# relife957/FastApriori

Measured on AMD Instinct MI355X. Metric: itemsets/sec (mining wall-clock), T10I4D100M min_sup=0.001, higher is better.
Workload: dtype int32/uint64-bitmap (exact integer counts); 1 GPU; model=T10I4D100M, global_batch=100000000, parallelism=dp1, n_itemsets=33139, min_count=100000

## Files before the change

csrc/hip/fa_hip.h:

```cpp
#pragma once
#include <hip/hip_runtime.h>
#include <stdint.h>

#define FA_API extern "C" __attribute__((visibility("default")))

#define FA_LAUNCH_RET() return (int)hipGetLastError()

namespace fa {

constexpr int kWave = 64;

__device__ __forceinline__ int lane_id() { return (int)(threadIdx.x & 63); }

__device__ __forceinline__ uint32_t popc64_acc(uint64_t x, uint32_t acc) {
  return acc + (uint32_t)__popc((uint32_t)x) + (uint32_t)__popc((uint32_t)(x >> 32));
}

__device__ __forceinline__ int wave_scan_incl_dpp(int v) {
  const int lane = (int)(threadIdx.x & 63);
  const int r = lane & 15;
  int t;
  t = __builtin_amdgcn_update_dpp(0, v, 0x111, 0xf, 0xf, false); if (r >= 1) v += t;
  t = __builtin_amdgcn_update_dpp(0, v, 0x112, 0xf, 0xf, false); if (r >= 2) v += t;
  t = __builtin_amdgcn_update_dpp(0, v, 0x114, 0xf, 0xf, false); if (r >= 4) v += t;
  t = __builtin_amdgcn_update_dpp(0, v, 0x118, 0xf, 0xf, false); if (r >= 8) v += t;
  t = __builtin_amdgcn_update_dpp(0, v, 0x142, 0xa, 0xf, false); if ((lane & 31) >= 16) v += t;
  t = __builtin_amdgcn_update_dpp(0, v, 0x143, 0xc, 0xf, false); if (lane >= 32) v += t;
  return v;
}

__device__ __forceinline__ int wave_last(int v) { return __builtin_amdgcn_readlane(v, 63); }

__device__ __forceinline__ uint32_t wave_sum_u32(uint32_t v) {
#pragma unroll
  for (int o = 32; o > 0; o >>= 1) v += __shfl_xor(v, o, 64);
  return v;
}

__device__ __forceinline__ unsigned long long wave_sum_u64(unsigned long long v) {
#pragma unroll
  for (int o = 32; o > 0; o >>= 1) v += __shfl_xor(v, o, 64);
  return v;
}

__device__ __forceinline__ int64_t wave_scan_incl_i64(int64_t v) {
  const int lane = (int)(threadIdx.x & 63);
#pragma unroll
  for (int o = 1; o < 64; o <<= 1) {
    const int64_t t = __shfl_up(v, o, 64);
    if (lane >= o) v += t;
  }
  return v;
}

__device__ __forceinline__ int wave_scan_incl(int v) { return wave_scan_incl_dpp(v); }
__device__ __forceinline__ int64_t wave_scan_incl(int64_t v) { return wave_scan_incl_i64(v); }
__device__ __forceinline__ int wave_sum(int v) { return (int)wave_sum_u32((uint32_t)v); }
__device__ __forceinline__ uint32_t wave_sum(uint32_t v) { return wave_sum_u32(v); }
__device__ __forceinline__ int64_t wave_sum(int64_t v) { return (int64_t)wave_sum_u64((unsigned long long)v); }


template <int W, int N, typename T, typename A>
__device__ __forceinline__ void wg_wave_prefix(const T (&x)[N], int src, T* scratch, A (&before)[N], A (&total)[N]) {
  const int lane = (int)(threadIdx.x & 63), w = (int)(threadIdx.x >> 6);
#pragma unroll
  for (int j = 0; j < N; ++j)
    if (lane == src) scratch[j * W + w] = x[j];
  __syncthreads();
#pragma unroll
  for (int j = 0; j < N; ++j) {
    A bef = 0, tot = 0;
#pragma unroll 4
    for (int k = 0; k < W; ++k) {
      const A t = (A)scratch[j * W + k];
      bef += k < w ? t : (A)0;
      tot += t;
    }
    before[j] = bef;
    total[j] = tot;
  }
}

template <int W, int N, typename T, typename A>
__device__ __forceinline__ void wg_scan_excl(const T (&v)[N], T* scratch, A (&excl)[N], A (&total)[N]) {
  T incl[N];
#pragma unroll
  for (int j = 0; j < N; ++j) incl[j] = wave_scan_incl(v[j]);
  wg_wave_prefix<W>(incl, 63, scratch, excl, total);
#pragma unroll
  for (int j = 0; j < N; ++j) excl[j] += (A)incl[j] - (A)v[j];
}

template <int W, typename T, typename A>
__device__ __forceinline__ A wg_scan_excl(T v, T* scratch, A& total) {
  const T v1[1] = {v};
  A e[1], t[1];
  wg_scan_excl<W>(v1, scratch, e, t);
  total = t[0];
  return e[0];
}

template <int W, int N, typename T>
__device__ __forceinline__ void wg_sum(const T (&v)[N], T* scratch, T (&total)[N]) {
  T s[N], before[N];
#pragma unroll
  for (int j = 0; j < N; ++j) s[j] = wave_sum(v[j]);
  wg_wave_prefix<W>(s, 0, scratch, before, total);
}

template <int W, typename T>
__device__ __forceinline__ T wg_sum(T v, T* scratch) {
  const T v1[1] = {v};
  T t[1];
  wg_sum<W>(v1, scratch, t);
  return t[0];
}

template <int W, int N, typename T, class Load, class Store>
__device__ __forceinline__ void wg_scan_chunks(int64_t n, int64_t (&carry)[N], T* scratch, Load&& load,
                                               Store&& store) {
  for (int64_t b0 = 0; b0 < n; b0 += 64 * W) {
    const int64_t i = b0 + threadIdx.x;
    T v[N];
#pragma unroll
    for (int j = 0; j < N; ++j) v[j] = 0;
    if (i < n) load(i, v);
    int64_t before[N], total[N];
    wg_scan_excl<W>(v, scratch, before, total);
#pragma unroll
    for (int j = 0; j < N; ++j) {
      before[j] += carry[j];
      carry[j] += total[j];
    }
    if (i < n) store(i, before, v);
    __syncthreads();
  }
}

template <int W, typename T, class Load, class Store>
__device__ __forceinline__ int64_t wg_scan_chunks(int64_t n, int64_t carry, T* scratch, Load&& load, Store&& store) {
  int64_t c[1] = {carry};
  wg_scan_chunks<W, 1>(
      n, c, scratch, [&](int64_t i, T (&v)[1]) { v[0] = load(i); },
      [&](int64_t i, const int64_t (&before)[1], const T (&v)[1]) { store(i, before[0], v[0]); });
  return c[0];
}

__device__ __forceinline__ void wave_lds_sync() {
  __builtin_amdgcn_wave_barrier();
  __asm__ __volatile__("" ::: "memory");
}

template <int U>
__device__ __forceinline__ void window_starts(unsigned long long* words, int srel, int q0,
                                              unsigned long long (&S)[U]) {
  const int lane = (int)(threadIdx.x & 63);
  if (lane < U) words[lane] = 0ull;
  wave_lds_sync();
  const int b = srel - q0;
  if (b >= 0 && b < 64 * U) atomicOr(&words[b >> 6], 1ull << (b & 63));
  wave_lds_sync();
#pragma unroll
  for (int u = 0; u < U; ++u) S[u] = words[u];
  wave_lds_sync();
}

__device__ __forceinline__ unsigned long long lanes_le_mask() {
  const int lane = (int)(threadIdx.x & 63);
  return lane == 63 ? ~0ull : ((2ull << lane) - 1);
}

__device__ __forceinline__ uint32_t xcd_remap(uint32_t orig, uint32_t nwg) {
  const uint32_t nx = 8;
  if (nwg < nx) return orig;
  uint32_t q = nwg / nx, r = nwg % nx, xcd = orig % nx;
  uint32_t base = xcd < r ? xcd * (q + 1) : r * (q + 1) + (xcd - r) * q;
  return base + orig / nx;
}

__device__ __forceinline__ int cmp_skip(const int32_t* __restrict__ a, const int32_t* __restrict__ s, int k,
                                        int p) {
  for (int i = 0, j = 0; i < k - 1; ++i, ++j) {
    if (j == p) ++j;
    const int32_t x = a[i], y = s[j];
    if (x != y) return x < y ? -1 : 1;
  }
  return 0;
}

struct DlDesc;

}

FA_API int fa_hip_dl_plan(const fa::DlDesc* desc, int L, long long* ctl, int F1, int32_t* item_map, void* rec,
                          int64_t max_pieces, int32_t* part, int64_t part_cap, int32_t* gpre, int64_t gpre_cap,
                          int sw, hipStream_t st);
FA_API int fa_hip_count_slab_rec_cls(const int64_t* roff, const int32_t* ranks, const int32_t* src, int64_t ncols,
                                     const int32_t* item_map, int F1, int n_used, const int32_t* gpre,
                                     const void* rec, int G, int C, const int32_t* wword, uint32_t* out, int sw,
                                     int n_wg, const uint64_t* bm, int64_t Wp, hipStream_t st,
                                     const int32_t* bm_rows, const int32_t* g_dev, int cls);
```

csrc/hip/prep.hip:

```cpp
#include "fa_hip.h"
#include "../host/fa_limits.h"

namespace fa {


template <bool kLds, bool kVec>
__global__ __launch_bounds__(256) void k_histogram(const int32_t* __restrict__ items, int64_t nnz,
                                                   int32_t V, int nrep, uint32_t* __restrict__ counts) {
  extern __shared__ uint32_t sh[];
  uint32_t* mine = sh;
  if (kLds) {
    for (int i = threadIdx.x; i < V * nrep; i += blockDim.x) sh[i] = 0;
    mine = sh + (nrep > 1 ? (threadIdx.x >> 6) % nrep : 0) * V;
    __syncthreads();
  }
  auto add = [&](int32_t v) {
    if (kLds) atomicAdd(&mine[v], 1u); else atomicAdd(&counts[v], 1u);
  };
  const int64_t stride = (int64_t)gridDim.x * blockDim.x;
  const int64_t gid = (int64_t)blockIdx.x * blockDim.x + threadIdx.x;
  const int64_t n4 = kVec ? (nnz >> 2) : 0;
  const int4* it4 = reinterpret_cast<const int4*>(items);
  for (int64_t i = gid; i < n4; i += stride) {
    int4 v = it4[i];
// ... 369 lines not shown
      for (int k = 0; k < 4; ++k) v[k] = v[k] >= 0 ? lut[v[k]] : -1;
#pragma unroll
      for (int k = 0; k < 4; ++k)
        if (v[k] >= 0) atomicOr(&b[v[k] >> 6], 1ull << (v[k] & 63));
    }
    wave_lds_sync();
    int base = 0;
    for (int m = 0; m < M; ++m) {
      const int widx = lane + 64 * m;
      unsigned long long word = b[widx];
      b[widx] = 0;
      const int c = __popcll(word);
      const int incl = wave_scan_incl_dpp(c);
      int64_t pos = o + base + incl - c;
      base += wave_last(incl);
      while (word) {
        ranks[pos++] = widx * 64 + (__ffsll((long long)word) - 1);
        word &= word - 1;
      }
    }
    wave_lds_sync();
  }
}

__device__ __forceinline__ uint64_t dmix64(uint64_t z) {
  z += 0x9E3779B97F4A7C15ull;
  z = (z ^ (z >> 30)) * 0xBF58476D1CE4E5B9ull;
  z = (z ^ (z >> 27)) * 0x94D049BB133111EBull;
  return z ^ (z >> 31);
}

__global__ __launch_bounds__(256) void k_row_hash(const int64_t* __restrict__ roff,
                                                  const int32_t* __restrict__ ranks, int64_t T,
                                                  int64_t* __restrict__ h1, int64_t* __restrict__ h2) {
  const int64_t x = (int64_t)blockIdx.x * blockDim.x + threadIdx.x;
  if (x >= T) return;
  uint64_t a = 0x243F6A8885A308D3ull, b = 0x13198A2E03707344ull;
  const int64_t s = roff[x], e = roff[x + 1];
  for (int64_t i = s; i < e; ++i) {
    uint64_t r = (uint32_t)ranks[i];
    a = dmix64(a ^ r);
    b = dmix64(b + r * 0xD6E8FEB86659FD93ull);
  }
  a = dmix64(a ^ (uint64_t)(e - s));
  h1[x] = (int64_t)(a >> 1);
  h2[x] = (int64_t)(b >> 1);
}

constexpr int kCmpProbeLen = 16;

constexpr uint32_t kNoSlot = 0xFFFFFFFFu;
constexpr int kProbeRange = 1 << 16;

__global__ __launch_bounds__(256) void k_dedup_probe(const int64_t* __restrict__ roff,
                                                     const int32_t* __restrict__ ranks,
                                                     const int64_t* __restrict__ T_dev, int64_t n_max,
                                                     uint32_t* __restrict__ slots, uint32_t* __restrict__ part) {
  const int64_t n = min(T_dev[0], n_max);
  const int64_t x = (int64_t)blockIdx.x * 256 + threadIdx.x;
  uint32_t slot = kNoSlot;
  if (x < n) {
    const int64_t s = roff[x], e = roff[x + 1];
    const int L = (int)(e - s);
    if (L <= kCmpProbeLen) {
      uint32_t v[kCmpProbeLen];
#pragma unroll
      for (int j = 0; j < kCmpProbeLen; ++j) v[j] = j < L ? (uint32_t)ranks[s + j] : 0u;
      uint64_t a = 0x243F6A8885A308D3ull;
#pragma unroll
      for (int j = 0; j < kCmpProbeLen; ++j)
        if (j < L) a = dmix64(a ^ (uint64_t)v[j]);
      a = dmix64(a ^ (uint64_t)L);
      slot = (uint32_t)((a >> 1) & (kProbeBits - 1));
    }
  }
  if (x < n_max) slots[x] = slot;
  __shared__ uint32_t wsum[4];
  const uint32_t c = wg_sum<4>(slot != kNoSlot ? 1u : 0u, wsum);
  if (threadIdx.x == 0) part[blockIdx.x] = c;
}

__global__ __launch_bounds__(1024) void k_probe_count(const uint32_t* __restrict__ slots, int64_t n_max,
                                                      const uint32_t* __restrict__ part, int nparts,
                                                      unsigned long long* __restrict__ out) {
  __shared__ uint32_t bits[kProbeRange / 32];
  __shared__ uint32_t wsum[2 * 16];
  for (int i = threadIdx.x; i < kProbeRange / 32; i += 1024) bits[i] = 0u;
  __syncthreads();
  const uint32_t lo = (uint32_t)blockIdx.x * kProbeRange;
  const uint4* s4 = reinterpret_cast<const uint4*>(slots);
  const int64_t n4 = n_max >> 2;
  auto mark = [&](uint32_t v) {
    const uint32_t d = v - lo;
    if (d < (uint32_t)kProbeRange) atomicOr(&bits[d >> 5], 1u << (d & 31));
  };
  constexpr int U = 8;
  int64_t i = threadIdx.x;
  for (; i + (U - 1) * 1024 < n4; i += U * 1024) {
    uint4 v[U];
#pragma unroll
    for (int k = 0; k < U; ++k) v[k] = s4[i + k * 1024];
#pragma unroll
    for (int k = 0; k < U; ++k) { mark(v[k].x); mark(v[k].y); mark(v[k].z); mark(v[k].w); }
  }
  for (; i < n4; i += 1024) {
    const uint4 v = s4[i];
    mark(v.x); mark(v.y); mark(v.z); mark(v.w);
  }
  for (int64_t j = (n4 << 2) + threadIdx.x; j < n_max; j += 1024) mark(slots[j]);
  __syncthreads();
  uint32_t c = 0, h = 0;
  for (int i = threadIdx.x; i < kProbeRange / 32; i += 1024) c += __popc(bits[i]);
  if (blockIdx.x == 0)
    for (int i = threadIdx.x; i < nparts; i += 1024) h += part[i];
  const uint32_t ch[2] = {c, h};
  uint32_t t[2];
  wg_sum<16>(ch, wsum, t);
  if (threadIdx.x == 0) {
    if (t[0]) atomicAdd(out, (unsigned long long)t[0]);
    if (blockIdx.x == 0) out[1] = t[1];
  }
}

__global__ __launch_bounds__(256) void k_build_bitmaps(
    const int64_t* __restrict__ roff, const int32_t* __restrict__ ranks, const int32_t* __restrict__ src,
    int64_t ncols, int32_t F1, int64_t Wp, int WT, int R, uint64_t* __restrict__ bm,
    const int32_t* __restrict__ item_map, const int32_t* __restrict__ used) {
  extern __shared__ uint32_t tile[];
  const int hw = 2 * WT;
  const int u0 = blockIdx.y * R;
  const int u1 = min(F1, u0 + R);
  const int nr = u1 - u0;
  const int r0 = item_map ? used[u0] : u0;
  const int r1 = item_map ? (u1 < F1 ? used[u1] : 0x7FFFFFFF) : u1;
  for (int i = threadIdx.x; i < nr * hw; i += blockDim.x) tile[i] = 0;
  __syncthreads();
  const int64_t c0 = (int64_t)blockIdx.x * WT * 64;
  for (int j = threadIdx.x; j < WT * 64; j += blockDim.x) {
    const int64_t c = c0 + j;
    if (c >= ncols) break;
    const int64_t row = src ? (int64_t)src[c] : c;
    if (row < 0) continue;
    int64_t s = roff[row];
    const int64_t e = roff[row + 1];
    int64_t lo = s, hi = e;
    while (lo < hi) {
      int64_t mid = (lo + hi) >> 1;
      if (ranks[mid] < r0) lo = mid + 1; else hi = mid;
    }
    const uint32_t bit = 1u << (j & 31);
    const int word = j >> 5;
    for (int64_t i = lo; i < e; ++i) {
      const int r = ranks[i];
      if (r >= r1) break;
      const int u = item_map ? item_map[r] : r;
      if (u >= 0) atomicOr(&tile[(u - u0) * hw + word], bit);
    }
  }
  __syncthreads();
  uint32_t* out = reinterpret_cast<uint32_t*>(bm);
  const int64_t base = c0 >> 5;
  for (int i = threadIdx.x; i < nr * hw; i += blockDim.x) {
    const int r = i / hw, w = i - r * hw;
    out[(int64_t)(u0 + r) * (2 * Wp) + base + w] = tile[i];
  }
}

__device__ __forceinline__ unsigned long long lane_range(int lo, int hi) {
  const unsigned long long h = hi >= 64 ? ~0ull : ((1ull << hi) - 1);
  const unsigned long long l = lo >= 64 ? ~0ull : ((1ull << lo) - 1);
  return hi > lo ? (h & ~l) : 0ull;
}

struct TrimWave {
  int64_t base;
  int n;
  int srel, erel;
};

__device__ __forceinline__ TrimWave trim_wave_setup(const int64_t* __restrict__ roff, int64_t row0, int64_t T) {
  const int lane = threadIdx.x & 63;
  TrimWave tw;
  tw.base = roff[row0];
  const int64_t end = roff[min(row0 + 64, T)];
  tw.n = (int)(end - tw.base);
  tw.srel = (int)(roff[min(row0 + lane, T)] - tw.base);
  tw.erel = (int)(roff[min(row0 + lane + 1, T)] - tw.base);
  return tw;
}

template <bool kLdsAlive>
__global__ __launch_bounds__(256) void k_trim_scan_count(const int64_t* __restrict__ roff,
                                                         const int32_t* __restrict__ ranks, int64_t T,
                                                         const int8_t* __restrict__ alive, int F1, int min_len,
                                                         const int32_t* __restrict__ wrow, int32_t* __restrict__ cnt,
                                                         int32_t* __restrict__ bk_rows, int32_t* __restrict__ bk_nnz) {
  extern __shared__ int8_t al[];
  __shared__ int wtot[4];
  if (kLdsAlive)
    for (int i = threadIdx.x; i < F1; i += blockDim.x) al[i] = alive[i];
  __syncthreads();
  const int8_t* A = kLdsAlive ? al : alive;
  const int lane = threadIdx.x & 63;
  const int64_t row0 = (int64_t)blockIdx.x * 256 + (threadIdx.x & ~63);
  const int64_t row = row0 + lane;
  int c = 0;
  if (row0 < T) {
    const TrimWave tw = trim_wave_setup(roff, row0, T);
    constexpr int U = 8;
    for (int p0 = 0; p0 < tw.n; p0 += 64 * U) {
      int32_t r[U];
#pragma unroll
      for (int u = 0; u < U; ++u) {
        const int p = p0 + 64 * u + lane;
        r[u] = p < tw.n ? ranks[tw.base + p] : 0;
      }
#pragma unroll
      for (int u = 0; u < U; ++u) {
        const int q0 = p0 + 64 * u;
        const unsigned long long b = __ballot(q0 + lane < tw.n && A[r[u]] != 0);
        c += __popcll(b & lane_range(max(tw.srel - q0, 0), min(max(tw.erel - q0, 0), 64)));
      }
    }
  }
  const bool keep = row < T && c >= min_len && (!wrow || wrow[row] > 0);
  if (row < T) cnt[row] = keep ? c : -1;
  int tr, tn;
  (void)wg_scan_excl<4>(keep ? 1 : 0, wtot, tr);
  __syncthreads();
  (void)wg_scan_excl<4>(keep ? c : 0, wtot, tn);
  __syncthreads();
  if (threadIdx.x == 0) { bk_rows[blockIdx.x] = tr; bk_nnz[blockIdx.x] = tn; }
}

template <bool kLdsAlive>
__global__ __launch_bounds__(256) void k_trim_emit(const int64_t* __restrict__ roff, const int32_t* __restrict__ ranks,
                                                   const int8_t* __restrict__ alive, int F1, int64_t T,
                                                   const int32_t* __restrict__ cnt, const int64_t* __restrict__ base_rows,
                                                   const int64_t* __restrict__ base_nnz, int64_t* __restrict__ nroff,
                                                   int32_t* __restrict__ nranks, int32_t* __restrict__ kept,
                                                   int64_t* __restrict__ hist) {
  extern __shared__ int8_t al[];
  __shared__ uint32_t hs[kTrimHist];
  __shared__ unsigned long long sw[4 * 4];
  __shared__ int wtot[4];
  if (kLdsAlive)
    for (int i = threadIdx.x; i < F1; i += blockDim.x) al[i] = alive[i];
  hs[threadIdx.x] = 0;
  const int8_t* A = kLdsAlive ? al : alive;
  const int lane = threadIdx.x & 63;
  const int64_t row0 = (int64_t)blockIdx.x * 256 + (threadIdx.x & ~63);
  const int64_t row = row0 + lane;
  const int32_t c = row < T ? cnt[row] : -1;
  const bool keep = c >= 0;
  int nk, nn;
  const int rk = wg_scan_excl<4>(keep ? 1 : 0, wtot, nk);
  __syncthreads();
  const int ok = wg_scan_excl<4>(keep ? c : 0, wtot, nn);
  __syncthreads();
  const int64_t obase = base_nnz[blockIdx.x] + ok;
  if (keep) {
    nroff[base_rows[blockIdx.x] + rk] = obase;
    kept[base_rows[blockIdx.x] + rk] = (int32_t)row;
    atomicAdd(&hs[min(c, kTrimHist - 1)], 1u);
  }
  if (row0 < T && __ballot(keep) != 0ull) {
    const TrimWave tw = trim_wave_setup(roff, row0, T);
    int64_t nxt = keep ? obase : -1;
    unsigned long long* words = sw + (threadIdx.x >> 6) * 4;
    const unsigned long long le = lanes_le_mask();
    int cs = 0;
    constexpr int U = 4;
    for (int p0 = 0; p0 < tw.n; p0 += 64 * U) {
      int32_t r[U];
#pragma unroll
      for (int u = 0; u < U; ++u) {
        const int p = p0 + 64 * u + lane;
        r[u] = p < tw.n ? ranks[tw.base + p] : 0;
      }
      unsigned long long S[U];
      window_starts<U>(words, tw.srel, p0, S);
#pragma unroll
      for (int u = 0; u < U; ++u) {
        const int q0 = p0 + 64 * u, p = q0 + lane;
        const bool a = p < tw.n && A[r[u]] != 0;
        const unsigned long long B = __ballot(a);
        const unsigned long long sle = S[u] & le;
        const int owner = cs + __popcll(sle) - 1;
        const int rs = sle ? 63 - __clzll(sle) : 0;
        const int64_t dst = __shfl(nxt, owner & 63, 64);
        if (a && dst >= 0) nranks[dst + __popcll(B & lane_range(rs, lane))] = r[u];
        if (nxt >= 0) nxt += __popcll(B & lane_range(max(tw.srel - q0, 0), min(max(tw.erel - q0, 0), 64)));
        cs += __popcll(S[u]);
      }
    }
  }
  __syncthreads();
  if (hist && hs[threadIdx.x])
    atomicAdd((unsigned long long*)&hist[(blockIdx.x & (kTrimStripes - 1)) * kTrimHist + threadIdx.x], (unsigned long long)hs[threadIdx.x]);
}


constexpr int kCmpPer = kCmpSpan / 256;
__device__ __forceinline__ bool cmp_stage(uint32_t* buf, const int32_t* __restrict__ items,
                                          const int32_t* __restrict__ lut, int64_t base, int64_t n_in) {
  if (n_in > kCmpSpan) return false;
  int32_t v[kCmpPer];
#pragma unroll
  for (int k = 0; k < kCmpPer; ++k) {
    const int64_t i = threadIdx.x + k * 256;
    v[k] = i < n_in ? items[base + i] : 0;
  }
#pragma unroll
  for (int k = 0; k < kCmpPer; ++k) {
    const int64_t i = threadIdx.x + k * 256;
    if (i < n_in) v[k] = lut[v[k]];
  }
#pragma unroll
  for (int k = 0; k < kCmpPer; ++k) {
    const int64_t i = threadIdx.x + k * 256;
    if (i < n_in) buf[i] = v[k] < 0 ? 0xFFFFFFFFu : (uint32_t)v[k];
  }
  return true;
}

constexpr int kCmpN = 16;
constexpr int kCmpMid = 64;

__device__ __forceinline__ bool cmp_mid(bool kept, int64_t L, bool staged) {
  const bool cand = kept && staged && L > kCmpN && L <= kCmpMid;
  const unsigned long long m = __ballot(cand);
  return cand && __popcll(m & (lanes_le_mask() >> 1)) < kCmpMidPerWave;
}

template <int KMAX>
__device__ __forceinline__ void wave_sort2(uint32_t& a, uint32_t& b) {
  const int lane = threadIdx.x & 63;
#pragma unroll
  for (int k = 2; k <= KMAX; k <<= 1) {
#pragma unroll
    for (int j = k >> 1; j > 0; j >>= 1) {
      const uint32_t oa = (uint32_t)__shfl_xor((int)a, j, 64);
      const uint32_t ob = (uint32_t)__shfl_xor((int)b, j, 64);
      const bool up = k == KMAX || (lane & k) == 0;
      const bool keep_min = up == ((lane & j) == 0);
      a = keep_min ? min(a, oa) : max(a, oa);
      b = keep_min ? min(b, ob) : max(b, ob);
    }
  }
}

__device__ __forceinline__ int nth_bit(unsigned long long m, int i) {
  for (; i > 0; --i) m &= m - 1;
  return __builtin_ctzll(m);
}

__device__ __forceinline__ unsigned long long blk_inc(uint32_t v) {
  return v == 0xFFFFFFFFu ? 0ull : 1ull << ((v >> 8) << 3);
}

__device__ __forceinline__ void cmp_block_totals(unsigned long long pc, int nb, int32_t* __restrict__ aggb) {
  __shared__ int bs[kCmpMaxNB][4];
  const int w = threadIdx.x >> 6, lane = threadIdx.x & 63;
#pragma unroll
  for (int b = 0; b < kCmpMaxNB; ++b) {
    if (b >= nb) break;
    const int t = wave_last(wave_scan_incl_dpp((int)((pc >> (8 * b)) & 255)));
    if (lane == 0) bs[b][w] = t;
  }
  __syncthreads();
  if ((int)threadIdx.x < nb)
    aggb[(int64_t)threadIdx.x * gridDim.x + blockIdx.x] =
        bs[threadIdx.x][0] + bs[threadIdx.x][1] + bs[threadIdx.x][2] + bs[threadIdx.x][3];
}

__global__ __launch_bounds__(256) void k_cmp_agg(const int64_t* __restrict__ off, const int32_t* __restrict__ items,
                                                 const int32_t* __restrict__ lut, int64_t n,
                                                 int32_t* __restrict__ agg, uint32_t* __restrict__ hist,
                                                 int32_t* __restrict__ aggb, int nb) {
  __shared__ uint32_t buf[kCmpSpan];
  __shared__ uint32_t lh[kCmpHist];
  __shared__ int sh[8];
  const int64_t r0 = (int64_t)blockIdx.x * 256, r1 = min(n, r0 + 256);
  const int64_t r = r0 + threadIdx.x;
  lh[threadIdx.x] = 0;
  const int64_t base = off[r0], n_in = off[r1] - base;
  const int64_t s = r < r1 ? off[r] : 0, e = r < r1 ? off[r + 1] : 0;
  const bool staged = cmp_stage(buf, items, lut, base, n_in);
  __syncthreads();
  int c = 0;
  unsigned long long pc = 0;
  for (int64_t i = s; i < e; ++i) {
    const uint32_t v = staged ? buf[i - base] : (uint32_t)lut[items[i]];
    c += v != 0xFFFFFFFFu;
    if (aggb) pc += blk_inc(v);
  }
  const int kept = c >= 2;
  if (aggb) cmp_block_totals(kept ? pc : 0ull, nb, aggb);
  const int kc[2] = {kept, kept ? c : 0};
  int ex[2], tot[2];
  wg_scan_excl<4>(kc, sh, ex, tot);
  if (kept) atomicAdd(&lh[min(c, kCmpHist - 1)], 1u);
  const bool mid = cmp_mid(kept, e - s, staged);
  const unsigned long long ob = __ballot(kept && e - s > kCmpN && !mid);
  __shared__ int ov_w[4];
  const int ovn[1] = {(int)__popcll(ob)};
  int ovp[1], ovt[1];
  wg_wave_prefix<4>(ovn, 0, ov_w, ovp, ovt);
  if (threadIdx.x == 0) {
    agg[3 * blockIdx.x] = tot[0]; agg[3 * blockIdx.x + 1] = tot[1];
    agg[3 * blockIdx.x + 2] = ovt[0];
  }
  if (lh[threadIdx.x]) atomicAdd(&hist[(blockIdx.x & (kCmpStripes - 1)) * kCmpHist + threadIdx.x], lh[threadIdx.x]);
}

__global__ __launch_bounds__(256) void k_cmp_emit(const int64_t* __restrict__ off, const int32_t* __restrict__ items,
                                                  const int32_t* __restrict__ lut, int64_t n,
                                                  const int64_t* __restrict__ pre_rows,
                                                  const int64_t* __restrict__ pre_items,
                                                  const int64_t* __restrict__ pre_over,
                                                  int32_t* __restrict__ kept_out, int64_t* __restrict__ roff,
                                                  int32_t* __restrict__ ranks, int32_t* __restrict__ over,
                                                  uint8_t* __restrict__ bcnt, int nb,
                                                  const int64_t* __restrict__ preb, uint8_t* __restrict__ lr,
                                                  int64_t lr_cap, int64_t* __restrict__ lbase,
                                                  int64_t* __restrict__ ovb) {
  constexpr int N = kCmpN;
  __shared__ uint32_t buf[kCmpSpan];
  __shared__ int sh[8];
  extern __shared__ int32_t tabx[];
  __shared__ int64_t wgb[kCmpMaxNB];
  const bool blk = bcnt != nullptr;
  const int64_t r0 = (int64_t)blockIdx.x * 256, r1 = min(n, r0 + 256);
  const int64_t r = r0 + threadIdx.x;
  const int64_t base = off[r0], n_in = off[r1] - base;
  const int64_t s = r < r1 ? off[r] : 0, e = r < r1 ? off[r + 1] : 0;
  const int64_t xr0 = pre_rows[blockIdx.x], obase = pre_items[blockIdx.x];
  const bool staged = cmp_stage(buf, items, lut, base, n_in);
  __syncthreads();
  const int64_t L = e - s;
  uint32_t a[N];
  int c = 0;
  unsigned long long pc = 0;
  if (L <= N) {
#pragma unroll
    for (int j = 0; j < N; ++j) {
      uint32_t v = 0xFFFFFFFFu;
      if (j < L) v = staged ? buf[s - base + j] : (uint32_t)lut[items[s + j]];
      a[j] = v;
      c += v != 0xFFFFFFFFu;
      if (blk) pc += blk_inc(v);
    }
  } else {
    for (int64_t i = s; i < e; ++i) {
      const uint32_t v = staged ? buf[i - base] : (uint32_t)lut[items[i]];
      c += v != 0xFFFFFFFFu;
      if (blk) pc += blk_inc(v);
    }
  }
  const int kept = c >= 2;
  const bool mid = cmp_mid(kept, L, staged);
  const int ov = kept && L > N && !mid;
  const int kc[2] = {kept, kept ? c : 0};
  int ex[2], tot[2];
  wg_scan_excl<4>(kc, sh, ex, tot);
  const int ea = ex[0], eb = ex[1], tb = tot[1];
  __shared__ int ov_w[4];
  const int w = threadIdx.x >> 6;
  const unsigned long long ob = __ballot(ov);
  const int ovn[1] = {(int)__popcll(ob)};
  int64_t ovp[1], ovt[1];
  wg_wave_prefix<4>(ovn, 0, ov_w, ovp, ovt);
  const int64_t ov_base = pre_over[blockIdx.x];
  const int64_t xk = xr0 + ea;
  int64_t ovi = -1;
  if (kept) {
    kept_out[xk] = (int32_t)r;
    roff[xk + 1] = obase + eb + c;
    if (ov) {
      ovi = ov_base + ovp[0] + __popcll(ob & (lanes_le_mask() >> 1));
      over[ovi] = (int32_t)xk;
    }
  }
  const bool mine = kept && L <= N;
  if (mine) bitonic_regs<N>(a);
  if (blk) {
    const int64_t bld = pre_rows[gridDim.x];
    const unsigned long long pk = kept ? pc : 0ull;
    const unsigned long long fpre = (pk << 8) * 0x0101010101010101ull;
    __shared__ int bs2[kCmpMaxNB][4];
    const int lane_ = threadIdx.x & 63;
    int exb[kCmpMaxNB];
#pragma unroll
    for (int b = 0; b < kCmpMaxNB; ++b) {
      exb[b] = 0;
      if (b < nb) {
        const int cb = (int)((pk >> (8 * b)) & 255);
        const int incl = wave_scan_incl_dpp(cb);
        exb[b] = incl - cb;
        if (lane_ == 63) bs2[b][w] = incl;
      }
    }
    if (lr && (int)threadIdx.x < nb) wgb[threadIdx.x] = preb[(int64_t)threadIdx.x * gridDim.x + blockIdx.x];
    __syncthreads();
#pragma unroll
    for (int b = 0; b < kCmpMaxNB; ++b) {
      if (b < nb) {
        for (int k = 0; k < w; ++k) exb[b] += bs2[b][k];
        if (kept) bcnt[(int64_t)b * bld + xk] = (uint8_t)(pk >> (8 * b));
        if (lr) {
          const int t = exb[b] - (int)((fpre >> (8 * b)) & 255);
          tabx[threadIdx.x * nb + b] = t;
          if (kept && (xk & 63) == 0) lbase[(int64_t)b * ((bld + 63) >> 6) + (xk >> 6)] = wgb[b] + exb[b];
          if (ovi >= 0) ovb[ovi * nb + b] = wgb[b] + t;
        }
      }
    }
    if (lr && mine) {
#pragma unroll
      for (int j = 0; j < N; ++j) {
        if (j < c) {
          const int b = (int)(a[j] >> 8);
          lr[wgb[b] + (int64_t)(tabx[threadIdx.x * nb + b] + j)] = (uint8_t)a[j];
        }
      }
    }
  }
  const int lane = threadIdx.x & 63;
  const unsigned long long m32 = __ballot(mid && L <= 32), m64 = __ballot(mid && L > 32);
  const int n32 = __popcll(m32), s32 = (n32 + 1) >> 1, nslot = s32 + __popcll(m64);
  auto slot_row = [&](int t) -> int {
    if (t < s32) {
      const int i = 2 * t + (lane >> 5);
      return i < n32 ? nth_bit(m32, i) : -1;
    }
    return t < nslot ? nth_bit(m64, t - s32) : -1;
  };
  uint32_t midv[kCmpMidPerWave];
#pragma unroll
  for (int t = 0; t < kCmpMidPerWave; ++t) {
    midv[t] = 0xFFFFFFFFu;
    if (t < nslot) {
      const int rw = slot_row(t);
      const int src = rw < 0 ? 0 : rw;
      const int idx = t < s32 ? (lane & 31) : lane;
      const int rs = __shfl((int)(s - base), src, 64);
      const int rl = __shfl((int)L, src, 64);
      if (rw >= 0 && idx < rl) midv[t] = buf[rs + idx];
    }
  }
#pragma unroll
  for (int t = 0; t < kCmpMidPerWave; t += 2) {
    if (t < nslot) {
      if (t + 1 < s32) {
        wave_sort2<32>(midv[t], midv[t + 1]);
      } else if (t >= s32) {
        wave_sort2<64>(midv[t], midv[t + 1]);
      } else {
        uint32_t none = 0xFFFFFFFFu;
        wave_sort2<32>(midv[t], none);
        if (t + 1 < nslot) wave_sort2<64>(midv[t + 1], none);
      }
    }
  }
  __syncthreads();
  if (staged && tb <= kCmpSpan) {
    if (mine) {
#pragma unroll
      for (int j = 0; j < N; ++j)
        if (j < c) buf[eb + j] = a[j];
    }
    {
#pragma unroll
      for (int t = 0; t < kCmpMidPerWave; ++t) {
        if (t < nslot) {
          const int rw = slot_row(t);
          const int src = rw < 0 ? 0 : rw;
          const int idx = t < s32 ? (lane & 31) : lane;
          const int rc = __shfl(c, src, 64), reb = __shfl(eb, src, 64);
          const bool in = rw >= 0 && idx < rc;
          if (in) {
            buf[reb + idx] = midv[t];
            if (lr) {
              const int b = (int)(midv[t] >> 8);
              lr[wgb[b] + (int64_t)(tabx[(w * 64 + rw) * nb + b] + idx)] = (uint8_t)midv[t];
            }
          }
        }
      }
    }
    __syncthreads();
    for (int i = threadIdx.x; i < tb; i += blockDim.x) ranks[obase + i] = (int32_t)buf[i];
  } else if (mine) {
#pragma unroll
    for (int j = 0; j < N; ++j)
      if (j < c) ranks[obase + eb + j] = (int32_t)a[j];
  }
}
__global__ __launch_bounds__(256) void k_block_counts_rows(const int64_t* __restrict__ roff,
                                                           const int32_t* __restrict__ ranks,
                                                           const int32_t* __restrict__ rows, int64_t nrows,
                                                           uint8_t* __restrict__ bcnt, int64_t bld, int nb,
                                                           const int8_t* __restrict__ flags) {
  const int64_t i = (int64_t)blockIdx.x * blockDim.x + threadIdx.x;
  if (i >= nrows || (flags && !flags[i])) return;
  const int64_t x = rows[i];
  int c[kCmpMaxNB] = {};
  for (int64_t k = roff[x], e = roff[x + 1]; k < e; ++k) {
    const int b = ranks[k] >> 8;
#pragma unroll
    for (int q = 0; q < kCmpMaxNB; ++q) c[q] += b == q;
  }
#pragma unroll
  for (int q = 0; q < kCmpMaxNB; ++q)
    if (q < nb) bcnt[(int64_t)q * bld + x] = (uint8_t)min(c[q], 255);
}

__global__ __launch_bounds__(256) void k_block_bsum(const uint8_t* __restrict__ bcnt, int64_t bld, int64_t T,
                                                    int nb, int64_t nbatch, int64_t* __restrict__ bsum) {
  const int64_t ng = (nbatch + 15) / 16;
  const int64_t t = (int64_t)blockIdx.x * 4 + (threadIdx.x >> 6);
  if (t >= nb * ng) return;
  const int lane = threadIdx.x & 63;
  const int64_t b = t / ng, q = (t - b * ng) * 16 + (lane >> 2);
  const int64_t x0 = q * 64 + 16 * (lane & 3);
  const uint8_t* src = bcnt + b * bld + x0;
  uint32_t s = 0;
  if (q < nbatch) {
    if (x0 + 16 <= T) {
      uint32_t acc = 0;
#pragma unroll
      for (int k = 0; k < 4; ++k) {
        uint32_t d;
        __builtin_memcpy(&d, src + 4 * k, 4);
        acc += (d & 0x00FF00FFu) + ((d >> 8) & 0x00FF00FFu);
      }
      s = (acc & 0xFFFFu) + (acc >> 16);
    } else {
      for (int k = 0; k < 16; ++k)
        if (x0 + k < T) s += src[k];
    }
  }
  s += (uint32_t)__builtin_amdgcn_mov_dpp((int)s, 0xB1, 0xf, 0xf, false);
  s += (uint32_t)__builtin_amdgcn_mov_dpp((int)s, 0x4E, 0xf, 0xf, false);
  if ((lane & 3) == 0 && q < nbatch) bsum[b * nbatch + q] = s;
}

}

using namespace fa;

FA_API int fa_hip_block_counts_rows(const int64_t* roff, const int32_t* ranks, const int32_t* rows, int64_t nrows,
                                    uint8_t* bcnt, int64_t bld, int nb, const int8_t* flags, hipStream_t st) {
  if (nrows <= 0) return 0;
  if (nb > kCmpMaxNB) return 1;
  hipLaunchKernelGGL(k_block_counts_rows, dim3((unsigned)((nrows + 255) / 256)), dim3(256), 0, st, roff, ranks, rows,
                     nrows, bcnt, bld, nb, flags);
  FA_LAUNCH_RET();
}

FA_API int fa_hip_block_bsum(const uint8_t* bcnt, int64_t bld, int64_t T, int nb, int64_t* bsum, hipStream_t st) {
  if (T <= 0) return 0;
  const int64_t nbatch = (T + 63) / 64;
  const int64_t ng = (nbatch + 15) / 16;
  hipLaunchKernelGGL(k_block_bsum, dim3((unsigned)((nb * ng + 3) / 4)), dim3(256), 0, st, bcnt, bld, T, nb,
                     nbatch, bsum);
  FA_LAUNCH_RET();
}

FA_API int fa_hip_histogram(const int32_t* items, int64_t nnz, int32_t V, uint32_t* counts,
                            hipStream_t st) {
  if (nnz <= 0) return 0;
  int64_t blocks = std::min<int64_t>((nnz + 256 * 16 - 1) / (256 * 16), 2048);
  const bool aligned = ((uintptr_t)items & 15) == 0;
  dim3 g((unsigned)blocks), b(256);
  if (V <= kLdsBins) {
    const int nrep = V * 4 <= kLdsBins / 4 ? 4 : 1;
    const size_t lds = (size_t)V * nrep * 4;
    if (aligned) hipLaunchKernelGGL((k_histogram<true, true>), g, b, lds, st, items, nnz, V, nrep, counts);
    else hipLaunchKernelGGL((k_histogram<true, false>), g, b, lds, st, items, nnz, V, nrep, counts);
  } else {
    if (aligned) hipLaunchKernelGGL((k_histogram<false, true>), g, b, 0, st, items, nnz, V, 1, counts);
    else hipLaunchKernelGGL((k_histogram<false, false>), g, b, 0, st, items, nnz, V, 1, counts);
  }
  FA_LAUNCH_RET();
}

FA_API int fa_hip_f1_rank(const int64_t* hist, int32_t V, int64_t thr, int numeric, int32_t* lut, int64_t* pack,
                          hipStream_t st) {
  if (V < 1 || V > kF1RankMax || thr < 1) return 1;
  hipLaunchKernelGGL(k_f1_rank, dim3((unsigned)((V + 255) / 256)), dim3(256), 0, st, hist, V, thr, numeric, lut, pack);
  FA_LAUNCH_RET();
}

__global__ __launch_bounds__(256) void k_txn_freq_count_wave(const int64_t* __restrict__ off,
                                                             const int32_t* __restrict__ items, int64_t n,
                                                             const int32_t* __restrict__ lut,
                                                             int32_t* __restrict__ cnt) {
  const int w = threadIdx.x >> 6, lane = threadIdx.x & 63;
  const int64_t nw = (int64_t)gridDim.x * 4;
  for (int64_t t = (int64_t)blockIdx.x * 4 + w; t < n; t += nw) {
    const int64_t s = off[t], L = off[t + 1] - s;
    int32_t c = 0;
    for (int64_t j0 = 0; j0 < L; j0 += 256) {
      int32_t v[4];
#pragma unroll
      for (int k = 0; k < 4; ++k) {
        const int64_t j = j0 + lane + 64 * k;
        v[k] = j < L ? items[s + j] : -1;
      }
#pragma unroll
      for (int k = 0; k < 4; ++k) c += __popcll(__ballot(v[k] >= 0 && lut[v[k]] >= 0));
    }
    if (lane == 0) cnt[t] = c;
  }
}

static int f1_grid(int64_t nnz) {
  return (int)std::max<int64_t>(1, std::min<int64_t>(kSkGridMax, (nnz + 1024 * 64 - 1) / (1024 * 64)));
}

FA_API int fa_hip_f1_sketch(const int32_t* items, int64_t nnz, uint32_t* partial, int* nwg, hipStream_t st) {
  const int g = f1_grid(nnz);
  *nwg = g;
  if (nnz <= 0) return 0;
  if (((uintptr_t)items & 15) == 0) hipLaunchKernelGGL(k_f1_sketch<true>, dim3(g), dim3(1024), 0, st, items, nnz, partial);
  else hipLaunchKernelGGL(k_f1_sketch<false>, dim3(g), dim3(1024), 0, st, items, nnz, partial);
  FA_LAUNCH_RET();
}

FA_API int fa_hip_f1_exact(const int32_t* items, int64_t nnz, const int32_t* keys, int log_s, uint32_t* counts,
                           hipStream_t st) {
  if (nnz <= 0) return 0;
  if (log_s < 6 || log_s > kSkLog) return 1;
  const int g = f1_grid(nnz);
  if (((uintptr_t)items & 15) == 0)
    hipLaunchKernelGGL(k_f1_exact<true>, dim3(g), dim3(1024), 0, st, items, nnz, keys, log_s, counts);
  else
    hipLaunchKernelGGL(k_f1_exact<false>, dim3(g), dim3(1024), 0, st, items, nnz, keys, log_s, counts);
  FA_LAUNCH_RET();
}

__global__ __launch_bounds__(256) void k_txn_freq_count_wv(const int64_t* __restrict__ off,
                                                           const int32_t* __restrict__ items, int64_t n,
                                                           const int32_t* __restrict__ lut, int32_t* __restrict__ cnt) {
  const int64_t q = (int64_t)blockIdx.x * 4 + (threadIdx.x >> 6);
  const int64_t x0 = q * 64;
  if (x0 >= n) return;
  const int lane = threadIdx.x & 63;
  const int64_t base = off[x0];
  const int nt = (int)(off[min(x0 + 64, n)] - base);
  const int srel = (int)(off[min(x0 + lane, n)] - base);
  const int erel = (int)(off[min(x0 + lane + 1, n)] - base);
  int c = 0;
  constexpr int U = 8;
  int v[U];
#pragma unroll
  for (int u = 0; u < U; ++u) v[u] = 64 * u + lane < nt ? items[base + 64 * u + lane] : -1;
  for (int p0 = 0; p0 < nt; p0 += 64 * U) {
    int nv[U];
#pragma unroll
    for (int u = 0; u < U; ++u) {
      const int p = p0 + 64 * (U + u) + lane;
      nv[u] = p < nt ? items[base + p] : -1;
    }
    int lv[U];
#pragma unroll
    for (int u = 0; u < U; ++u) lv[u] = v[u] >= 0 ? lut[v[u]] : -1;
#pragma unroll
    for (int u = 0; u < U; ++u) {
      const bool f = lv[u] >= 0;
      const unsigned long long b = __ballot(f);
      const int lo = max(srel - (p0 + 64 * u), 0), hi = min(erel - (p0 + 64 * u), 64);
      if (hi > lo) {
        const unsigned long long m = (hi >= 64 ? ~0ull : ((1ull << hi) - 1)) & ~((1ull << lo) - 1);
        c += __popcll(b & m);
      }
    }
#pragma unroll
    for (int u = 0; u < U; ++u) v[u] = nv[u];
  }
  if (x0 + lane < n) cnt[x0 + lane] = c;
}

FA_API int fa_hip_txn_freq_count(const int64_t* off, const int32_t* items, int64_t n, int64_t nnz,
                                 const int32_t* lut, int32_t* cnt, hipStream_t st) {
  if (n <= 0) return 0;
  if (nnz > 8 * n && nnz <= 48 * n) {
    hipLaunchKernelGGL(k_txn_freq_count_wv, dim3((unsigned)((n + 255) / 256)), dim3(256), 0, st, off, items, n, lut,
                       cnt);
    FA_LAUNCH_RET();
  }
  if (nnz > 48 * n)
    hipLaunchKernelGGL(k_txn_freq_count_wave, dim3((unsigned)std::min<int64_t>((n + 3) / 4, 8192)), dim3(256), 0, st,
                       off, items, n, lut, cnt);
  else if (nnz > 8 * n)
    hipLaunchKernelGGL(k_txn_freq_count_span<16384>, dim3((unsigned)((n + 255) / 256)), dim3(256), 0, st, off, items,
                       n, lut, cnt);
  else
    hipLaunchKernelGGL(k_txn_freq_count, dim3((unsigned)((n + 255) / 256)), dim3(256), 0, st, off, items, n, lut, cnt);
  FA_LAUNCH_RET();
}

FA_API int fa_hip_compress_regs(int tier, const int64_t* off, const int32_t* items, const int32_t* lut,
                                const int32_t* rows, int64_t nrows, const int32_t* kept,
                                const int64_t* roff, int32_t* ranks, int8_t* over_flag, hipStream_t st) {
  if (nrows <= 0) return 0;
  dim3 g((unsigned)((nrows + 255) / 256));
  if (tier == 16)
    hipLaunchKernelGGL(k_compress_regs<16>, g, dim3(256), 0, st, off, items, lut, rows, nrows, kept, roff, ranks, over_flag);
  else if (tier == 32)
    hipLaunchKernelGGL(k_compress_regs<32>, g, dim3(256), 0, st, off, items, lut, rows, nrows, kept, roff, ranks, over_flag);
  else if (tier == 64)
    hipLaunchKernelGGL(k_compress_regs<64>, g, dim3(256), 0, st, off, items, lut, rows, nrows, kept, roff, ranks, over_flag);
  else
    return 1;
  FA_LAUNCH_RET();
}

FA_API int fa_hip_compress_regs_bc(const int64_t* off, const int32_t* items, const int32_t* lut, const int32_t* rows,
                                   int64_t nrows, const int32_t* kept, const int64_t* roff, int32_t* ranks,
                                   int8_t* over_flag, uint8_t* bcnt, int64_t bld, int nb, hipStream_t st) {
  if (nrows <= 0) return 0;
  if (nb < 1 || nb > kCmpMaxNB) return 1;
  hipLaunchKernelGGL(k_compress_regs<64>, dim3((unsigned)((nrows + 255) / 256)), dim3(256), 0, st, off, items, lut,
                     rows, nrows, kept, roff, ranks, over_flag, bcnt, bld, nb);
  FA_LAUNCH_RET();
}

FA_API int fa_hip_compress_staged(const int64_t* off, const int32_t* items, const int32_t* lut, int64_t T,
                                  const int32_t* kept, const int64_t* roff, int32_t* ranks, int8_t* over_flag,
                                  hipStream_t st) {
  if (T <= 0) return 0;
  hipLaunchKernelGGL(k_compress_staged<16>, dim3((unsigned)((T + 255) / 256)), dim3(256), 0, st, off, items, lut,
                     T, kept, roff, ranks, over_flag);
  FA_LAUNCH_RET();
}

FA_API int fa_hip_compress_staged64(const int64_t* off, const int32_t* items, const int32_t* lut, int64_t T,
                                    const int32_t* kept, const int64_t* roff, int32_t* ranks, int8_t* over_flag,
                                    int F1, hipStream_t st) {
  if (T <= 0) return 0;
  const dim3 g((unsigned)((T + 255) / 256));
  if (F1 > 0 && F1 < 0xFFFF)
    hipLaunchKernelGGL((k_compress_staged<64, 16384, uint16_t>), g, dim3(256), 0, st, off, items, lut, T, kept, roff,
                       ranks, over_flag);
  else
    hipLaunchKernelGGL((k_compress_staged<64, 16384>), g, dim3(256), 0, st, off, items, lut, T, kept, roff, ranks,
                       over_flag);
  FA_LAUNCH_RET();
}

FA_API int fa_hip_compress_lds(const int64_t* off, const int32_t* items, const int32_t* lut,
                               const int32_t* rows, int64_t nrows, const int32_t* kept,
                               const int64_t* roff, int32_t* ranks, int32_t* too_long,
                               int32_t* n_too_long, hipStream_t st) {
  if (nrows <= 0) return 0;
  hipLaunchKernelGGL(k_compress_lds, dim3((unsigned)nrows), dim3(256), 0, st, off, items, lut, rows, kept, roff, ranks, too_long, n_too_long);
  FA_LAUNCH_RET();
}

FA_API int fa_hip_compress_wave(const int64_t* off, const int32_t* items, const int32_t* lut, const int32_t* rows,
                                int64_t nrows, const int32_t* kept, const int64_t* roff, int32_t* ranks, int F1,
                                const int8_t* flags, hipStream_t st) {
  if (nrows <= 0) return 0;
  const int M = (F1 + 4095) / 4096;
  if (F1 > kCwMaxF1) return 1;
  const int64_t g = std::min<int64_t>((nrows + 3) / 4, 8192);
  hipLaunchKernelGGL(k_compress_wave, dim3((unsigned)g), dim3(256), 0, st, off, items, lut, rows, nrows, kept, roff,
                     ranks, std::max(M, 1), flags);
  FA_LAUNCH_RET();
}

// ... 187 lines not shown
```

Before: 903,800 itemsets/s.

## Pack compaction scans into bit-fields and keep small-block scatter offsets in registers

In the staged path, the kept flag, overflow flag, item count and per-block byte counts are packed into a few 32-bit words. Each word is scanned once with a DPP wave scan, which replaces several separate workgroup scans, their barriers and the per-block scan loop. Row loads become branchless reads of a 16-wide padded LDS row, and per-block counts use a packed 6-bit popcount trick when there are at most 4 blocks. Scatter offsets for that case stay in registers instead of tabx shared memory. The change adds bit-width constraints enforced by static asserts, extra padding in the LDS buffer, and more code paths to keep correct.

New measurement: 908,600 itemsets/s, median of 6. Within noise of the previous version (+0.5%).

```diff
diff --git a/csrc/hip/fa_hip.h b/csrc/hip/fa_hip.h
--- a/csrc/hip/fa_hip.h
+++ b/csrc/hip/fa_hip.h
@@ -30,6 +30,17 @@
 }
 
 __device__ __forceinline__ int wave_last(int v) { return __builtin_amdgcn_readlane(v, 63); }
+
+__device__ __forceinline__ uint32_t wave_scan_incl_packed(uint32_t x) {
+  int v = (int)x;
+  v += __builtin_amdgcn_update_dpp(0, v, 0x111, 0xf, 0xf, false);
+  v += __builtin_amdgcn_update_dpp(0, v, 0x112, 0xf, 0xf, false);
+  v += __builtin_amdgcn_update_dpp(0, v, 0x114, 0xf, 0xf, false);
+  v += __builtin_amdgcn_update_dpp(0, v, 0x118, 0xf, 0xf, false);
+  v += __builtin_amdgcn_update_dpp(0, v, 0x142, 0xa, 0xf, false);
+  v += __builtin_amdgcn_update_dpp(0, v, 0x143, 0xc, 0xf, false);
+  return (uint32_t)v;
+}
 
 __device__ __forceinline__ uint32_t wave_sum_u32(uint32_t v) {
 #pragma unroll
diff --git a/csrc/hip/prep.hip b/csrc/hip/prep.hip
--- a/csrc/hip/prep.hip
+++ b/csrc/hip/prep.hip
@@ -695,29 +695,46 @@
 
 
 constexpr int kCmpPer = kCmpSpan / 256;
+constexpr int kCmpN = 16;
+constexpr int kCmpBuf = kCmpSpan + kCmpN;
 __device__ __forceinline__ bool cmp_stage(uint32_t* buf, const int32_t* __restrict__ items,
                                           const int32_t* __restrict__ lut, int64_t base, int64_t n_in) {
   if (n_in > kCmpSpan) return false;
+  if (n_in <= 0) return true;
+  const int32_t* __restrict__ src = items + base;
+  const uint32_t last = (uint32_t)n_in - 1u;
   int32_t v[kCmpPer];
 #pragma unroll
-  for (int k = 0; k < kCmpPer; ++k) {
-    const int64_t i = threadIdx.x + k * 256;
-    v[k] = i < n_in ? items[base + i] : 0;
-  }
-#pragma unroll
-  for (int k = 0; k < kCmpPer; ++k) {
-    const int64_t i = threadIdx.x + k * 256;
-    if (i < n_in) v[k] = lut[v[k]];
-  }
-#pragma unroll
-  for (int k = 0; k < kCmpPer; ++k) {
-    const int64_t i = threadIdx.x + k * 256;
-    if (i < n_in) buf[i] = v[k] < 0 ? 0xFFFFFFFFu : (uint32_t)v[k];
-  }
+  for (int k = 0; k < kCmpPer; ++k)
+    if (256u * k <= last) v[k] = src[min((uint32_t)threadIdx.x + 256u * k, last)];
+#pragma unroll
+  for (int k = 0; k < kCmpPer; ++k)
+    if (256u * k <= last) v[k] = lut[v[k]];
+#pragma unroll
+  for (int k = 0; k < kCmpPer; ++k)
+    if (256u * k <= last) buf[threadIdx.x + 256 * k] = v[k] < 0 ? 0xFFFFFFFFu : (uint32_t)v[k];
   return true;
 }
 
-constexpr int kCmpN = 16;
+__device__ __forceinline__ void cmp_row16(const uint32_t* buf, int s0, int L, uint32_t (&a)[kCmpN]) {
+  const uint32_t* p = buf + (L > 0 ? s0 : 0);
+  uint32_t v[kCmpN];
+#pragma unroll
+  for (int j = 0; j < kCmpN; ++j) v[j] = p[j];
+  const uint32_t m = 0xFFFFFFFFu << L;
+#pragma unroll
+  for (int j = 0; j < kCmpN; ++j) a[j] = v[j] | (uint32_t)((int32_t)(m << (31 - j)) >> 31);
+}
+
+__device__ __forceinline__ uint32_t cmp_count16(const uint32_t (&a)[kCmpN]) {
+  uint32_t pc = 0;
+#pragma unroll
+  for (int j = 0; j < kCmpN; ++j) pc += 1u << (min(a[j] >> 8, 4u) * 6u);
+  return pc;
+}
+__device__ __forceinline__ unsigned long long cmp_count16_bytes(uint32_t pc) {
+  return (unsigned long long)((pc & 63u) | ((pc >> 6) & 63u) << 8 | ((pc >> 12) & 63u) << 16 | ((pc >> 18) & 63u) << 24);
+}
 constexpr int kCmpMid = 64;
 
 __device__ __forceinline__ bool cmp_mid(bool kept, int64_t L, bool staged) {
@@ -752,6 +769,44 @@
   return v == 0xFFFFFFFFu ? 0ull : 1ull << ((v >> 8) << 3);
 }
 
+constexpr int kCmpWords = 1 + kCmpMaxNB / 2;
+constexpr int kCmpWStride = 8;
+static_assert(kCmpSpan < (1 << 13), "word 0 of the packed scan: kept items in 13 bits");
+static_assert(kCmpSpan < (1 << 16) && kCmpWords <= kCmpWStride, "block-count pairs of the packed scan");
+
+__device__ __forceinline__ uint32_t cmp_word0(int kept, int ov, int c) {
+  return (uint32_t)kept | (uint32_t)ov << 9 | (uint32_t)(kept ? c : 0) << 18;
+}
+__device__ __forceinline__ uint32_t cmp_pair(unsigned long long pk, int k) {
+  const uint32_t h = (uint32_t)(pk >> (16 * k));
+  return (h & 255u) | (h & 0xFF00u) << 8;
+}
+
+__device__ __forceinline__ void cmp_scan_packed(const uint32_t (&x)[kCmpWords], int nw, uint32_t (*sc)[kCmpWStride],
+                                                uint32_t (&excl)[kCmpWords], uint32_t& tot0) {
+  const int lane = (int)(threadIdx.x & 63);
+  const int w = __builtin_amdgcn_readfirstlane((int)(threadIdx.x >> 6));
+#pragma unroll
+  for (int i = 0; i < kCmpWords; ++i) {
+    excl[i] = 0;
+    if (i < nw) {
+      const uint32_t incl = wave_scan_incl_packed(x[i]);
+      if (lane == 63) sc[w][i] = incl;
+      excl[i] = incl - x[i];
+    }
+  }
+  __syncthreads();
+  tot0 = sc[0][0] + sc[1][0] + sc[2][0] + sc[3][0];
+#pragma unroll
+  for (int k = 0; k < 3; ++k) {
+    if (k < w) {
+#pragma unroll
+      for (int i = 0; i < kCmpWords; ++i)
+        if (i < nw) excl[i] += sc[k][i];
+    }
+  }
+}
+
 __device__ __forceinline__ void cmp_block_totals(unsigned long long pc, int nb, int32_t* __restrict__ aggb) {
   __shared__ int bs[kCmpMaxNB][4];
   const int w = threadIdx.x >> 6, lane = threadIdx.x & 63;
@@ -771,9 +826,10 @@
                                                  const int32_t* __restrict__ lut, int64_t n,
                                                  int32_t* __restrict__ agg, uint32_t* __restrict__ hist,
                                                  int32_t* __restrict__ aggb, int nb) {
-  __shared__ uint32_t buf[kCmpSpan];
+  __shared__ uint32_t buf[kCmpBuf];
   __shared__ uint32_t lh[kCmpHist];
   __shared__ int sh[8];
+  __shared__ __attribute__((aligned(16))) uint32_t sc[4][kCmpWStride];
   const int64_t r0 = (int64_t)blockIdx.x * 256, r1 = min(n, r0 + 256);
   const int64_t r = r0 + threadIdx.x;
   lh[threadIdx.x] = 0;
@@ -789,20 +845,45 @@
     if (aggb) pc += blk_inc(v);
   }
   const int kept = c >= 2;
-  if (aggb) cmp_block_totals(kept ? pc : 0ull, nb, aggb);
-  const int kc[2] = {kept, kept ? c : 0};
-  int ex[2], tot[2];
-  wg_scan_excl<4>(kc, sh, ex, tot);
   if (kept) atomicAdd(&lh[min(c, kCmpHist - 1)], 1u);
   const bool mid = cmp_mid(kept, e - s, staged);
-  const unsigned long long ob = __ballot(kept && e - s > kCmpN && !mid);
-  __shared__ int ov_w[4];
-  const int ovn[1] = {(int)__popcll(ob)};
-  int ovp[1], ovt[1];
-  wg_wave_prefix<4>(ovn, 0, ov_w, ovp, ovt);
-  if (threadIdx.x == 0) {
-    agg[3 * blockIdx.x] = tot[0]; agg[3 * blockIdx.x + 1] = tot[1];
-    agg[3 * blockIdx.x + 2] = ovt[0];
+  const int ov = kept && e - s > kCmpN && !mid;
+  if (staged) {
+    const unsigned long long pk = kept ? pc : 0ull;
+    const int nw = aggb ? 1 + ((nb + 1) >> 1) : 1;
+    const int w = __builtin_amdgcn_readfirstlane((int)(threadIdx.x >> 6));
+#pragma unroll
+    for (int i = 0; i < kCmpWords; ++i) {
+      if (i < nw) {
+        const uint32_t t = wave_scan_incl_packed(i == 0 ? cmp_word0(kept, ov, c) : cmp_pair(pk, i - 1));
+        if ((threadIdx.x & 63) == 63) sc[w][i] = t;
+      }
+    }
+    __syncthreads();
+    if (threadIdx.x == 0) {
+      const uint32_t t = sc[0][0] + sc[1][0] + sc[2][0] + sc[3][0];
+      agg[3 * blockIdx.x] = (int32_t)(t & 511u); agg[3 * blockIdx.x + 1] = (int32_t)(t >> 18);
+      agg[3 * blockIdx.x + 2] = (int32_t)((t >> 9) & 511u);
+    }
+    if (aggb && (int)threadIdx.x < nb) {
+      const int i = 1 + ((int)threadIdx.x >> 1);
+      const uint32_t t = sc[0][i] + sc[1][i] + sc[2][i] + sc[3][i];
+      aggb[(int64_t)threadIdx.x * gridDim.x + blockIdx.x] = (int32_t)((t >> (16 * (threadIdx.x & 1))) & 0xFFFFu);
+    }
+  } else {
+    if (aggb) cmp_block_totals(kept ? pc : 0ull, nb, aggb);
+    const int kc[2] = {kept, kept ? c : 0};
+    int ex[2], tot[2];
+    wg_scan_excl<4>(kc, sh, ex, tot);
+    const unsigned long long ob = __ballot(ov);
+    __shared__ int ov_w[4];
+    const int ovn[1] = {(int)__popcll(ob)};
+    int ovp[1], ovt[1];
+    wg_wave_prefix<4>(ovn, 0, ov_w, ovp, ovt);
+    if (threadIdx.x == 0) {
+      agg[3 * blockIdx.x] = tot[0]; agg[3 * blockIdx.x + 1] = tot[1];
+      agg[3 * blockIdx.x + 2] = ovt[0];
+    }
   }
   if (lh[threadIdx.x]) atomicAdd(&hist[(blockIdx.x & (kCmpStripes - 1)) * kCmpHist + threadIdx.x], lh[threadIdx.x]);
 }
@@ -819,16 +900,19 @@
                                                   int64_t lr_cap, int64_t* __restrict__ lbase,
                                                   int64_t* __restrict__ ovb) {
   constexpr int N = kCmpN;
-  __shared__ uint32_t buf[kCmpSpan];
+  __shared__ uint32_t buf[kCmpBuf];
   __shared__ int sh[8];
+  __shared__ __attribute__((aligned(16))) uint32_t sc[4][kCmpWStride];
   extern __shared__ int32_t tabx[];
   __shared__ int64_t wgb[kCmpMaxNB];
   const bool blk = bcnt != nullptr;
+  const bool small = blk && nb <= 4;
   const int64_t r0 = (int64_t)blockIdx.x * 256, r1 = min(n, r0 + 256);
   const int64_t r = r0 + threadIdx.x;
   const int64_t base = off[r0], n_in = off[r1] - base;
   const int64_t s = r < r1 ? off[r] : 0, e = r < r1 ? off[r + 1] : 0;
   const int64_t xr0 = pre_rows[blockIdx.x], obase = pre_items[blockIdx.x];
+  if (lr && (int)threadIdx.x < nb) wgb[threadIdx.x] = preb[(int64_t)threadIdx.x * gridDim.x + blockIdx.x];
   const bool staged = cmp_stage(buf, items, lut, base, n_in);
   __syncthreads();
   const int64_t L = e - s;
@@ -836,13 +920,22 @@
   int c = 0;
   unsigned long long pc = 0;
   if (L <= N) {
-#pragma unroll
-    for (int j = 0; j < N; ++j) {
-      uint32_t v = 0xFFFFFFFFu;
-      if (j < L) v = staged ? buf[s - base + j] : (uint32_t)lut[items[s + j]];
-      a[j] = v;
-      c += v != 0xFFFFFFFFu;
-      if (blk) pc += blk_inc(v);
+    if (staged) {
+      cmp_row16(buf, (int)(s - base), (int)L, a);
+    } else {
+#pragma unroll
+      for (int j = 0; j < N; ++j) a[j] = j < L ? (uint32_t)lut[items[s + j]] : 0xFFFFFFFFu;
+    }
+    if (small) {
+      const uint32_t p6 = cmp_count16(a);
+      c = N - (int)(p6 >> 24);
+      pc = cmp_count16_bytes(p6);
+    } else {
+#pragma unroll
+      for (int j = 0; j < N; ++j) {
+        c += a[j] != 0xFFFFFFFFu;
+        if (blk) pc += blk_inc(a[j]);
+      }
     }
   } else {
     for (int64_t i = s; i < e; ++i) {
@@ -854,16 +947,50 @@
   const int kept = c >= 2;
   const bool mid = cmp_mid(kept, L, staged);
   const int ov = kept && L > N && !mid;
-  const int kc[2] = {kept, kept ? c : 0};
-  int ex[2], tot[2];
-  wg_scan_excl<4>(kc, sh, ex, tot);
-  const int ea = ex[0], eb = ex[1], tb = tot[1];
-  __shared__ int ov_w[4];
+  const unsigned long long pk = kept ? pc : 0ull;
   const int w = threadIdx.x >> 6;
-  const unsigned long long ob = __ballot(ov);
-  const int ovn[1] = {(int)__popcll(ob)};
-  int64_t ovp[1], ovt[1];
-  wg_wave_prefix<4>(ovn, 0, ov_w, ovp, ovt);
+  int ea, eb, tb, ovx;
+  int exb[kCmpMaxNB];
+  if (staged) {
+    uint32_t x[kCmpWords], ex[kCmpWords], t0;
+    x[0] = cmp_word0(kept, ov, c);
+#pragma unroll
+    for (int k = 0; k < kCmpMaxNB / 2; ++k) x[1 + k] = cmp_pair(pk, k);
+    cmp_scan_packed(x, blk ? 1 + ((nb + 1) >> 1) : 1, sc, ex, t0);
+    ea = (int)(ex[0] & 511u); ovx = (int)((ex[0] >> 9) & 511u); eb = (int)(ex[0] >> 18);
+    tb = (int)(t0 >> 18);
+#pragma unroll
+    for (int b = 0; b < kCmpMaxNB; ++b) exb[b] = (int)((ex[1 + (b >> 1)] >> (16 * (b & 1))) & 0xFFFFu);
+  } else {
+    const int kc[2] = {kept, kept ? c : 0};
+    int ex[2], tot[2];
+    wg_scan_excl<4>(kc, sh, ex, tot);
+    ea = ex[0]; eb = ex[1]; tb = tot[1];
+    __shared__ int ov_w[4];
+    const unsigned long long ob = __ballot(ov);
+    const int ovn[1] = {(int)__popcll(ob)};
+    int ovp[1], ovt[1];
+    wg_wave_prefix<4>(ovn, 0, ov_w, ovp, ovt);
+    ovx = ovp[0] + (int)__popcll(ob & (lanes_le_mask() >> 1));
+    __shared__ int bs2[kCmpMaxNB][4];
+#pragma unroll
+    for (int b = 0; b < kCmpMaxNB; ++b) {
+      exb[b] = 0;
+      if (blk && b < nb) {
+        const int cb = (int)((pk >> (8 * b)) & 255);
+        const int incl = wave_scan_incl_dpp(cb);
+        exb[b] = incl - cb;
+        if ((threadIdx.x & 63) == 63) bs2[b][w] = incl;
+      }
+    }
+    if (blk) {
+      __syncthreads();
+#pragma unroll
+      for (int b = 0; b < kCmpMaxNB; ++b)
+        if (b < nb)
+          for (int k = 0; k < w; ++k) exb[b] += bs2[b][k];
+    }
+  }
   const int64_t ov_base = pre_over[blockIdx.x];
   const int64_t xk = xr0 + ea;
   int64_t ovi = -1;
@@ -871,7 +998,7 @@
     kept_out[xk] = (int32_t)r;
     roff[xk + 1] = obase + eb + c;
     if (ov) {
-      ovi = ov_base + ovp[0] + __popcll(ob & (lanes_le_mask() >> 1));
+      ovi = ov_base + ovx;
       over[ovi] = (int32_t)xk;
     }
   }
@@ -879,42 +1006,46 @@
   if (mine) bitonic_regs<N>(a);
   if (blk) {
     const int64_t bld = pre_rows[gridDim.x];
-    const unsigned long long pk = kept ? pc : 0ull;
-    const unsigned long long fpre = (pk << 8) * 0x0101010101010101ull;
-    __shared__ int bs2[kCmpMaxNB][4];
-    const int lane_ = threadIdx.x & 63;
-    int exb[kCmpMaxNB];
-#pragma unroll
-    for (int b = 0; b < kCmpMaxNB; ++b) {
-      exb[b] = 0;
-      if (b < nb) {
-        const int cb = (int)((pk >> (8 * b)) & 255);
-        const int incl = wave_scan_incl_dpp(cb);
-        exb[b] = incl - cb;
-        if (lane_ == 63) bs2[b][w] = incl;
-      }
-    }
-    if (lr && (int)threadIdx.x < nb) wgb[threadIdx.x] = preb[(int64_t)threadIdx.x * gridDim.x + blockIdx.x];
-    __syncthreads();
+    const unsigned long long fpre = small ? (unsigned long long)(((uint32_t)pk << 8) * 0x01010101u)
+                                          : (pk << 8) * 0x0101010101010101ull;
+    const bool regs = small && lr_cap <= 0x7FFFFFFFll;
+    int tq[4] = {0, 0, 0, 0};
 #pragma unroll
     for (int b = 0; b < kCmpMaxNB; ++b) {
       if (b < nb) {
-        for (int k = 0; k < w; ++k) exb[b] += bs2[b][k];
         if (kept) bcnt[(int64_t)b * bld + xk] = (uint8_t)(pk >> (8 * b));
         if (lr) {
           const int t = exb[b] - (int)((fpre >> (8 * b)) & 255);
-          tabx[threadIdx.x * nb + b] = t;
+          if (b < 4) tq[b] = t;
+          if (mid || !regs) tabx[threadIdx.x * nb + b] = t;
           if (kept && (xk & 63) == 0) lbase[(int64_t)b * ((bld + 63) >> 6) + (xk >> 6)] = wgb[b] + exb[b];
           if (ovi >= 0) ovb[ovi * nb + b] = wgb[b] + t;
         }
       }
     }
     if (lr && mine) {
-#pragma unroll
-      for (int j = 0; j < N; ++j) {
-        if (j < c) {
-          const int b = (int)(a[j] >> 8);
-          lr[wgb[b] + (int64_t)(tabx[threadIdx.x * nb + b] + j)] = (uint8_t)a[j];
+      if (regs) {
+        uint32_t d[4];
+#pragma unroll
+        for (int b = 0; b < 4; ++b) d[b] = (uint32_t)wgb[b] + (uint32_t)(tq[b] + N);
+#pragma unroll
+        for (int j = 0; j < N; ++j) {
+          if (j < c) {
+            const uint32_t v = a[j];
+            uint32_t q = d[0];
+            q = v >= 256u ? d[1] : q;
+            q = v >= 512u ? d[2] : q;
+            q = v >= 768u ? d[3] : q;
+            lr[(int64_t)(uint64_t)q + (j - N)] = (uint8_t)v;
+          }
+        }
+      } else {
+#pragma unroll
+        for (int j = 0; j < N; ++j) {
+          if (j < c) {
+            const int b = (int)(a[j] >> 8);
+            lr[wgb[b] + (int64_t)(tabx[threadIdx.x * nb + b] + j)] = (uint8_t)a[j];
+          }
         }
       }
     }
@@ -960,8 +1091,7 @@
   if (staged && tb <= kCmpSpan) {
     if (mine) {
 #pragma unroll
-      for (int j = 0; j < N; ++j)
-        if (j < c) buf[eb + j] = a[j];
+      for (int j = 0; j < N; ++j) buf[(j < c ? eb : kCmpSpan) + j] = a[j];
     }
     {
 #pragma unroll
```
